# sjulier/Refactored_ORB_SLAM2

Measured on AMD Instinct MI355X. Metric: frames/s (extract+match) at KITTI 1241×376, 2000 feat; 1/2/4/8 GPU + CPU ref, higher is better.
Workload: dtype u8; 1 GPU; kitti_stereo_1241x376_2000feat_8lvl: 2x ORBextractor + ComputeStereoMatches + SearchByProjection(cur,last); parallelism=frame-shard x1, collective=none, driver=torch, queries=one pass: orbfe_track_queries_stereo_device

## Files before the change

refactored_orb_slam2_amd/csrc/match_kernels.hip:

```cpp
#include <string.h>
#include <atomic>
#include <mutex>

#include "match_internal.h"

#define WAVE 64

__device__ __forceinline__ int hamming256(const uint4 a0, const uint4 a1, const uint4 b0, const uint4 b1) {
  return __popc(a0.x ^ b0.x) + __popc(a0.y ^ b0.y) + __popc(a0.z ^ b0.z) + __popc(a0.w ^ b0.w) +
         __popc(a1.x ^ b1.x) + __popc(a1.y ^ b1.y) + __popc(a1.z ^ b1.z) + __popc(a1.w ^ b1.w);
}
__device__ __forceinline__ void load_desc(const uint8_t* p, uint4& d0, uint4& d1) {
  const uint4* q = reinterpret_cast<const uint4*>(p);
  d0 = q[0];
  d1 = q[1];
}
__device__ __forceinline__ void load_desc4(const uint8_t* p, uint4& d0, uint4& d1) {
  const uint32_t* q = reinterpret_cast<const uint32_t*>(p);
  d0 = make_uint4(q[0], q[1], q[2], q[3]);
  d1 = make_uint4(q[4], q[5], q[6], q[7]);
}

__device__ __forceinline__ unsigned wave_min_u32(unsigned v) {
#define ORBFE_MIN_STEP(ctrl, rmask) v = min(v, (unsigned)__builtin_amdgcn_update_dpp((int)0xffffffff, (int)v, ctrl, rmask, 0xf, false))
// ... 1089 lines not shown
      const int maxr = (int)ceilf(kp.y + r), minr = (int)floorf(kp.y - r);
      int b0 = max(minr, 0) >> 3, b1 = min(maxr >> 3, nb - 1);
      if (b1 - b0 >= STEREO_BUCKET_SPAN) b1 = b0 + STEREO_BUCKET_SPAN - 1;
      for (int b = b0; b <= b1; b++) {
        const int key = b * nl + oct;
        const int pos = atomicAdd(&cnt[key], 1);
        if (pass == 1) bi[start[key] + pos] = make_int4(iR, __float_as_int(kp.x), __float_as_int(kp.y), kp.octave);
      }
    }
    __syncthreads();
    if (pass == 0) {
      const int per = (nk + 255) / 256;
      const int k0 = min(tid * per, nk), k1 = min(k0 + per, nk);
      int sum = 0;
      for (int k = k0; k < k1; k++) sum += cnt[k];
      part[tid] = sum;
      __syncthreads();
      if (tid == 0) {
        int run = 0;
        for (int i = 0; i < 256; i++) { const int v = part[i]; part[i] = run; run += v; }
        start[nk] = run;
      }
      __syncthreads();
      int run = part[tid];
      for (int k = k0; k < k1; k++) { start[k] = run; run += cnt[k]; }
      __syncthreads();
      for (int b = tid; b <= nk; b += 256) bs[b] = start[b];
      for (int b = tid; b < nk; b += 256) cnt[b] = 0;
      __syncthreads();
    }
  }
}

__device__ __forceinline__ unsigned sad_u32(unsigned a, unsigned b, unsigned c) {
  unsigned r;
  asm("v_sad_u32 %0, %1, %2, %3" : "=v"(r) : "v"(a), "v"(b), "v"(c));
  return r;
}
#define ORBFE_ROW_ALL(op, v) do { \
    v = op(v, (unsigned)__builtin_amdgcn_update_dpp(0, (int)v, 0x128, 0xf, 0xf, false));  \
    v = op(v, (unsigned)__builtin_amdgcn_update_dpp(0, (int)v, 0x124, 0xf, 0xf, false));  \
    v = op(v, (unsigned)__builtin_amdgcn_update_dpp(0, (int)v, 0x122, 0xf, 0xf, false));  \
    v = op(v, (unsigned)__builtin_amdgcn_update_dpp(0, (int)v, 0x121, 0xf, 0xf, false));  \
  } while (0)
__device__ __forceinline__ unsigned op_min_u(unsigned a, unsigned b) { return min(a, b); }
__device__ __forceinline__ unsigned op_add_u(unsigned a, unsigned b) { return a + b; }
__device__ __forceinline__ unsigned op_or_u(unsigned a, unsigned b) { return a | b; }
__device__ __forceinline__ unsigned row_min_u32(unsigned v) { ORBFE_ROW_ALL(op_min_u, v); return v; }
__device__ __forceinline__ unsigned row_sum_u32(unsigned v) { ORBFE_ROW_ALL(op_add_u, v); return v; }
__device__ __forceinline__ unsigned row_or_u32(unsigned v) { ORBFE_ROW_ALL(op_or_u, v); return v; }

struct SmLevel {
  const uint8_t* baseL; const uint8_t* baseR;
  unsigned long long strideL, strideR;
  int pitchL, pitchR, wL, hL, wR, hR;
  float scale, inv_scale;
  int tiledL, tiledR;
};
#define SM_G 16
#define SM_KPB (256 / SM_G)
#ifndef SM_ROUNDS
#define SM_ROUNDS 2
#endif
#ifndef SM_SAD_T
#define SM_SAD_T 8
#endif
#define SAD_LP 32
#define SAD_RP 48
#define SAD_WIN (11 * SAD_LP + 11 * SAD_RP + 16)
#ifndef SM_XCD_PAIRS
#define SM_XCD_PAIRS 1
#endif
__global__ __launch_bounds__(256) void stereo_match_kernel(StereoParams P) {
  int pair = blockIdx.y, bx = blockIdx.x;
#if SM_XCD_PAIRS
  {
    const unsigned gx = gridDim.x;
    const unsigned lin = blockIdx.y * gx + blockIdx.x;
    const unsigned g8 = lin / (8u * gx);
    if (8u * g8 + 8u <= gridDim.y) {
      const unsigned within = lin - g8 * 8u * gx;
      pair = (int)(8u * g8 + (within & 7u));
      bx = (int)(within >> 3);
    }
  }
#endif
  const int lane = threadIdx.x & (WAVE - 1);
  const int sub = lane & (SM_G - 1);
  const int grp = threadIdx.x / SM_G;
  const int iL = bx * SM_KPB + grp;
  __shared__ SmLevel s_lv[ORBFE_MAX_LEVELS];
  __shared__ float s_r[ORBFE_MAX_LEVELS];
  __shared__ __attribute__((aligned(16))) uint8_t sad_win[SM_KPB][SAD_WIN];
  __shared__ uint16_t s_offL[128], s_offR[128];
  if (threadIdx.x >= 128) {
    const unsigned p = threadIdx.x - 128, yy = p / 11u, xx = p - yy * 11u;
    s_offL[p] = (uint16_t)(p < 121 ? yy * SAD_LP + xx : 0);
    s_offR[p] = (uint16_t)(p < 121 ? yy * SAD_RP + xx : 0);
  }
  if (threadIdx.x < ORBFE_MAX_LEVELS) {
    const int l = threadIdx.x;
    const bool in = l < P.n_levels;
    SmLevel v;
    v.baseL = P.pyrL.base[l] + (size_t)pair * P.pyrL.img_stride[l];
    v.baseR = P.pyrR.base[l] + (size_t)pair * P.pyrR.img_stride[l];
    v.strideL = 0; v.strideR = 0;
    v.pitchL = P.pyrL.pitch[l]; v.pitchR = P.pyrR.pitch[l];
    v.wL = in ? P.pyrL.w[l] : 0; v.hL = in ? P.pyrL.h[l] : 0;
    v.wR = in ? P.pyrR.w[l] : 0; v.hR = in ? P.pyrR.h[l] : 0;
    v.scale = P.scale[l]; v.inv_scale = P.inv_scale[l];
    v.tiledL = (int)((P.pyrL.tiled >> l) & 1u); v.tiledR = (int)((P.pyrR.tiled >> l) & 1u);
    s_lv[l] = v;
    s_r[l] = 2.0f * P.scale[l];
  }
  __syncthreads();
  const int cap = P.cap, nl = P.n_levels;
  float* out_ur = P.u_right + (size_t)pair * cap;
  float* out_depth = P.depth + (size_t)pair * cap;
  int32_t* out_sad = P.sad + (size_t)pair * cap;
  const orbfe_keypoint* kl = P.kpsL + (size_t)pair * cap;
  const uint8_t* dl = P.descL + (size_t)pair * cap * 32;
  const uint8_t* dr = P.descR + (size_t)pair * cap * 32;
  const int nL = P.nL[pair];
  const int iLc = min(iL, cap - 1);
  const float uL = kl[iLc].x, vL = kl[iLc].y;
  const int octL = kl[iLc].octave;
  uint4 a0, a1;
  load_desc(dl + (size_t)iLc * 32, a0, a1);
  if (sub == 0 && iL < cap) { out_ur[iL] = -1.0f; out_depth[iL] = -1.0f; out_sad[iL] = -1; }
  const int levelL = min(max(octL, 0), nl - 1);
  const int nRows = P.pyrL.h[0];
  const int row = (int)vL;
// ... 32 lines not shown
      if (__ballot(ok[r]) != 0ull) {
        const unsigned key = ((unsigned)hamming256(a0, a1, b0[r], b1[r]) << 16) | (unsigned)rec[r].x;
        if (ok[r] && key < best) {
          best = key;
          best_x = rx[r];
        }
      }
    }
  }
  {
    const unsigned k = ((best >> 16) < (unsigned)ORBFE_TH_HIGH) ? best : 0xFFFFFFFFu;
    best = row_min_u32(k);
    best_x = __int_as_float((int)row_or_u32((k == best && k != 0xFFFFFFFFu) ? (unsigned)__float_as_int(best_x) : 0u));
  }
  const float uR0 = best_x;
  const int thOrbDist = (ORBFE_TH_HIGH + ORBFE_TH_LOW) / 2;
  act = act && best != 0xFFFFFFFFu && (int)(best >> 16) < thOrbDist;
  if (__ballot(act) == 0ull) return;

  const SmLevel lv = s_lv[levelL];
  const float sfac = lv.inv_scale;
  const float scaleduL = roundf(uL * sfac);
  const float scaledvL = roundf(vL * sfac);
  const float scaleduR0 = roundf(uR0 * sfac);
  const int w = 5, L = 5;
  const float iniu = scaleduR0 + L - w;
  const float endu = scaleduR0 + L + w + 1;
  act = act && !(iniu < 0 || endu >= (float)lv.wR);
  const int yW = (int)(scaledvL - w), xW = (int)(scaleduL - w), xRc = (int)scaleduR0;
  const int xR0 = xRc - L - w;
  act = act && !(yW < 0 || yW + 2 * w >= lv.hL || xW < 0 || xW + 2 * w >= lv.wL || xR0 < 0 || xRc + L + w >= lv.wR ||
                 yW + 2 * w >= lv.hR);
  if (__ballot(act) == 0ull) return;
  uint8_t* winL = &sad_win[grp][0];
  uint8_t* winR = winL + 11 * SAD_LP;
  const int axL = xW & ~15, axR = xR0 & ~15;
  if (act && sub < 11) {
    typedef const __attribute__((address_space(1))) uint8_t* gptr_t;
    typedef unsigned int u32x4 __attribute__((ext_vector_type(4)));
    const int y = yW + sub;
    u32x4 vl[2], vr[3];
#pragma unroll
    for (int k = 0; k < 2; k++) {
      const int x = min(axL + 16 * k, lv.pitchL - 16);
      vl[k] = *reinterpret_cast<const __attribute__((address_space(1))) u32x4*>((gptr_t)(uintptr_t)lv.baseL + orbfe_level_offset(x, y, lv.pitchL, lv.tiledL != 0));
    }
#pragma unroll
    for (int k = 0; k < 3; k++) {
      const int x = min(axR + 16 * k, lv.pitchR - 16);
      vr[k] = *reinterpret_cast<const __attribute__((address_space(1))) u32x4*>((gptr_t)(uintptr_t)lv.baseR + orbfe_level_offset(x, y, lv.pitchR, lv.tiledR != 0));
    }
    u32x4* wl = reinterpret_cast<u32x4*>(winL + sub * SAD_LP);
    wl[0] = vl[0]; wl[1] = vl[1];
    u32x4* wr = reinterpret_cast<u32x4*>(winR + sub * SAD_RP);
    wr[0] = vr[0]; wr[1] = vr[1]; wr[2] = vr[2];
  }
  __builtin_amdgcn_fence(__ATOMIC_RELEASE, "wavefront");
  __builtin_amdgcn_wave_barrier();
  __builtin_amdgcn_fence(__ATOMIC_ACQUIRE, "wavefront");
  const uint8_t* WL = winL + (xW - axL);
  const uint8_t* WR = winR + (xR0 - axR);
  const int cLm = (int)WL[w * SAD_LP + w] - 255;
  int cRm[11];
#pragma unroll
  for (int k = 0; k < 11; k++) cRm[k] = (int)WR[w * SAD_RP + w + k] - 255;
  unsigned acc[11];
#pragma unroll
  for (int k = 0; k < 11; k++) acc[k] = 0;
#pragma unroll
  for (int t = 0; t < SM_SAD_T; t++) {
    const int p = sub + SM_G * t;
    if (t < 7 || p < 121) {
      const unsigned a = (unsigned)((int)WL[s_offL[p]] - cLm);
      const uint8_t* rrow = WR + s_offR[p];
#pragma unroll
      for (int k = 0; k < 11; k++) acc[k] = sad_u32(a, (unsigned)((int)rrow[k] - cRm[k]), acc[k]);
    }
  }
  unsigned pk[6];
#pragma unroll
  for (int j = 0; j < 5; j++) pk[j] = acc[2 * j] | (acc[2 * j + 1] << 16);
  pk[5] = acc[10];
#pragma unroll
  for (int j = 0; j < 6; j++) pk[j] = row_sum_u32(pk[j]);
  unsigned mine = pk[0];
  {
    const int t = sub >> 1;
    mine = t == 1 ? pk[1] : mine; mine = t == 2 ? pk[2] : mine; mine = t == 3 ? pk[3] : mine;
    mine = t == 4 ? pk[4] : mine; mine = t == 5 ? pk[5] : mine;
    mine = (sub & 1) ? (mine >> 16) : (mine & 0xffffu);
  }
  const unsigned kmin = row_min_u32(sub < 11 ? ((mine << 4) | (unsigned)sub) : 0xFFFFFFFFu);
  const int bk = (int)(kmin & 15u);
  const int sadBest = (int)(kmin >> 4);
  const int bestincR = bk - L;
  const int rowbase = lane & ~(SM_G - 1);
  const int i1 = __builtin_amdgcn_ds_bpermute((rowbase + ((bk + 15) & 15)) << 2, (int)mine);
  const int i3 = __builtin_amdgcn_ds_bpermute((rowbase + ((bk + 1) & 15)) << 2, (int)mine);
  const int i2 = sadBest;
  if (!act || sub != 0 || bestincR == -L || bestincR == L) return;
  const float dist1 = (float)i1, dist2 = (float)i2, dist3 = (float)i3;
  const float deltaR = (dist1 - dist3) / (2.0f * (dist1 + dist3 - 2.0f * dist2));
  if (deltaR < -1 || deltaR > 1) return;
  float bestuR = lv.scale * ((float)scaleduR0 + (float)bestincR + deltaR);
  float disparity = (uL - bestuR);
  if (disparity >= minD && disparity < maxD) {
    if (disparity <= 0) {
      disparity = (float)0.01;
      bestuR = (float)((double)uL - 0.01);
    }
    out_depth[iL] = P.mbf / disparity;
    out_ur[iL] = bestuR;
    out_sad[iL] = sadBest;
  }
}

__global__ __launch_bounds__(256) void stereo_median_kernel(StereoParams P) {
// ... 137 lines not shown
```

refactored_orb_slam2_amd/csrc/extract_kernels.hip:

```cpp
#include <stdlib.h>
#include <string.h>

#include "orbfe_internal.h"
#include "../../include/orb_pattern_data.h"

#define WAVE 64

__device__ __forceinline__ int wave_incl_scan(int v) {
  v += __builtin_amdgcn_update_dpp(0, v, 0x111, 0xf, 0xf, false);
  v += __builtin_amdgcn_update_dpp(0, v, 0x112, 0xf, 0xf, false);
  v += __builtin_amdgcn_update_dpp(0, v, 0x114, 0xf, 0xf, false);
  v += __builtin_amdgcn_update_dpp(0, v, 0x118, 0xf, 0xf, false);
  v += __builtin_amdgcn_update_dpp(0, v, 0x142, 0xa, 0xf, false);
  v += __builtin_amdgcn_update_dpp(0, v, 0x143, 0xc, 0xf, false);
  return v;
}

template <int T>
__device__ __forceinline__ int block_incl_scan_t(int v, int* tmp, int* total) {
  const int tid = threadIdx.x;
  const int lane = tid & (WAVE - 1), wid = tid >> 6;
  int s = wave_incl_scan(v);
  if (T == WAVE) {
    *total = __builtin_amdgcn_readlane(s, WAVE - 1);
// ... 2006 lines not shown
  }
  const double r = x * 0x1.45F306DC9C883p+23;
  const int n = ((int32_t)r + 0x800000) >> 24;
  x = x - (double)n * 0x1.921FB54442D18p0;
  const double s = ((n + 1) & 2) ? -1.0 : 1.0;
  const bool flip = (n & 2) != 0;
  const double xs = x * s, x2 = x * x;
  *sn = sc_poly(xs, x2, n, flip);
  *cs = sc_poly(xs, x2, n ^ 1, flip);
}

#ifndef ORI_PITCH
#define ORI_PITCH 48
#endif
#ifndef DSC_PITCH
#define DSC_PITCH 64
#endif
template <int PITCH>
__device__ __forceinline__ void patch_store16(uint8_t* base, int r, int c, const uint4& v) {
  if constexpr (PITCH % 16 == 0) {
    *reinterpret_cast<uint4*>(base + r * PITCH + 16 * c) = v;
  } else {
    uint32_t* q = reinterpret_cast<uint32_t*>(base + r * PITCH + 16 * c);
    q[0] = v.x; q[1] = v.y; q[2] = v.z; q[3] = v.w;
  }
}
#define ORI_BYTES ((31 * ORI_PITCH + 15) & ~15)
#ifndef OD_DMA_STAGE
#define OD_DMA_STAGE 1
#endif
#define OD_BUF (37 * DSC_PITCH)
#if OD_DMA_STAGE
#define PATCH_BYTES (2 * OD_BUF)
#define OD_DMA(gsrc, lds_dst) do { \
    unsigned keep_m0; \
    asm volatile("s_mov_b32 %0, m0\n\ts_mov_b32 m0, %2\n\ts_nop 0\n\tglobal_load_lds_dwordx4 %1, off\n\ts_mov_b32 m0, %0" \
                 : "=&s"(keep_m0) : "v"(gsrc), "s"(lds_dst) : "memory"); \
  } while (0)
#else
#define PATCH_BYTES ((ORI_BYTES + 37 * DSC_PITCH + 15) & ~15)
#endif

#ifndef OD_K
#define OD_K 8
#ifndef OD_DSC_NARROW
#define OD_DSC_NARROW 1
#endif
#endif
#ifndef OD_FAKE_TILED_RAW
#define OD_FAKE_TILED_RAW 0
#endif
#ifndef OD_FAKE_TABLES
#define OD_FAKE_TABLES 0
#endif
#if FC_TIMING
__device__ unsigned long long g_od_prof[4096 * 8];
extern "C" int orbfe_debug_od_profile(unsigned long long* out, int reset) {
  static unsigned long long h[4096 * 8];
  if (hipMemcpyFromSymbol(h, HIP_SYMBOL(g_od_prof), sizeof(h)) != hipSuccess) return 1;
  for (int i = 0; i < 8; i++) out[i] = 0;
  for (int sl = 0; sl < 4096; sl++)
    for (int i = 0; i < 8; i++) out[i] += h[sl * 8 + i];
  if (reset) { memset(h, 0, sizeof(h)); if (hipMemcpyToSymbol(HIP_SYMBOL(g_od_prof), h, sizeof(h)) != hipSuccess) return 1; }
  return 0;
}
#endif
__device__ __attribute__((aligned(16))) uint32_t g_ic_w[256 * 2];
#ifndef OD_WGS
#define OD_WGS 7
#endif
__global__ __launch_bounds__(256, OD_WGS) void orient_describe8_kernel(DescribeParams P) {
  __shared__ __attribute__((aligned(16))) uint8_t patch[4][PATCH_BYTES];
  const int lane = threadIdx.x & (WAVE - 1);
  const int wv_id = __builtin_amdgcn_readfirstlane((int)(threadIdx.x >> 6));
  int bx = blockIdx.x, img = blockIdx.y;
  if (P.xcd_images) {
    const unsigned gx = gridDim.x;
    const unsigned lin = blockIdx.y * gx + blockIdx.x;
    const unsigned grp = lin / (8u * gx);
    if (8u * grp + 8u <= gridDim.y) {
      const unsigned within = lin - grp * 8u * gx;
      img = (int)(8u * grp + (within & 7u));
      bx = (int)(within >> 3);
    }
  }
#if FC_TIMING
  uint32_t tacc0 = 0, tacc1 = 0, tacc2 = 0, tacc3 = 0, tacc4 = 0, tacc5 = 0, tprev = (uint32_t)__builtin_readcyclecounter();
#endif
  const int s0 = (bx * 4 + wv_id) * OD_K;
  const int32_t* ln = P.lvl_n + (size_t)img * ORBFE_MAX_LEVELS;
  if (s0 >= P.kp_per_image) return;
  const int ln_lane = lane < P.n_levels ? ln[lane] : 0;
  const int slot_c = min(s0 + (lane & (OD_K - 1)), P.kp_per_image - 1);
  const uint32_t e_lane = P.lvl_kp[(size_t)img * P.kp_per_image + slot_c];
  float4 pk[4];
#pragma unroll
#if OD_FAKE_TABLES
  for (int r = 0; r < 4; r++) pk[r] = make_float4((float)(lane & 7) - 3.f, (float)(r * 2 + (lane >> 4)) - 5.f, (float)(lane & 15) - 8.f, (float)(r) - 2.f);
#else
  for (int r = 0; r < 4; r++) pk[r] = *reinterpret_cast<const float4*>(&g_pattern_f[(r * 64 + lane) * 4]);
#endif
  uint32_t wu[4], wv[4];
#pragma unroll
  for (int j = 0; j < 4; j++) {
    const int it = lane + WAVE * j;
#if OD_FAKE_TABLES
    wu[j] = 0x01020304u * (uint32_t)(it & 7); wv[j] = 0x01010101u * (uint32_t)(it >> 3);
#else
    const uint2 w2 = reinterpret_cast<const uint2*>(g_ic_w)[it];
    wu[j] = w2.x; wv[j] = w2.y;
#endif
  }
#if !OD_DMA_STAGE
  uint8_t* ori = &patch[wv_id][0];
  uint8_t* dsc = ori + ORI_BYTES;
#endif

  int i_out = -1, i_level = 0, i_cx = 0, i_cy = 0, i_score = 0;
  {
    const int slot = s0 + lane;
    int level = 0, off_level = 0;
    for (int l = 1; l < P.n_levels; l++) {
      const bool ge = slot >= P.kp_off[l];
      level += ge ? 1 : 0;
      off_level = ge ? P.kp_off[l] : off_level;
    }
    const int idx = slot - off_level;
    int out = idx, ln_level = 0;
    for (int l = 0; l < P.n_levels; l++) {
      const int lnl = __builtin_amdgcn_readlane(ln_lane, l);
      out += l < level ? lnl : 0;
      ln_level = l == level ? lnl : ln_level;
    }
    if (lane < OD_K && slot < P.kp_per_image && idx < ln_level && out < P.cap) {
      const uint32_t e = e_lane;
      i_out = out; i_level = level;
      i_cx = (int)(e & 0xfff) + ORBFE_EDGE; i_cy = (int)((e >> 12) & 0xfff) + ORBFE_EDGE; i_score = (int)(e >> 24);
    }
    if (s0 == 0 && lane == 0) {
      int tot = 0;
      for (int l = 0; l < P.n_levels; l++) tot += __builtin_amdgcn_readlane(ln_lane, l);
      P.out_n[img] = tot;
    }
  }
  const unsigned valid_mask = (unsigned)(__ballot(i_out >= 0) & ((1ull << OD_K) - 1ull));
  if (valid_mask == 0) return;
  FC_T(0);

#if OD_DSC_NARROW && !OD_DMA_STAGE
  int r3[3], c3[3];
#pragma unroll
  for (int j = 0; j < 3; j++) { const int i = lane + WAVE * j; r3[j] = i / 3; c3[j] = i - 3 * r3[j]; }
#endif
#if !OD_DMA_STAGE
  auto issue_ori = [&](int k, uint4 vo[2]) {
    const int level = __builtin_amdgcn_readlane(i_level, k), cx = __builtin_amdgcn_readlane(i_cx, k), cy = __builtin_amdgcn_readlane(i_cy, k);
    const int pitch = P.pyr.pitch[level];
    const uint8_t* plane = P.pyr.base[level] + (size_t)img * P.pyr.img_stride[level];
    const int ax_o = (cx - 15) & ~15;
// ... 3 lines not shown
      const int r = i / 3, c = i - r * 3;
#if OD_FAKE_TILED_RAW
      (void)pitch; (void)plane;
      vo[j] = i < 31 * 3 ? *reinterpret_cast<const uint4*>(P.blur.base[level] + (size_t)img * P.blur.img_stride[level] + blur_tiled_offset(ax_o + 16 * c, cy - 15 + r, P.blur.pitch[level])) : make_uint4(0, 0, 0, 0);
#else
      vo[j] = i < 31 * 3 ? *reinterpret_cast<const uint4*>(plane + orbfe_level_offset(ax_o + 16 * c, cy - 15 + r, pitch, (P.pyr.tiled >> level) & 1u)) : make_uint4(0, 0, 0, 0);
#endif
    }
  };
  auto issue_dsc = [&](int k, uint4 vd[3]) {
    const int level = __builtin_amdgcn_readlane(i_level, k), cx = __builtin_amdgcn_readlane(i_cx, k), cy = __builtin_amdgcn_readlane(i_cy, k);
    const int bpitch = P.blur.pitch[level];
    const uint8_t* bplane = P.blur.base[level] + (size_t)img * P.blur.img_stride[level];
    const int ax_d = (cx - 18) & ~15;
#if OD_DSC_NARROW
    const bool wide = ((cx - 18) & 15) > 11;
    const int n_pieces = wide ? 37 * 4 : 37 * 3;
#pragma unroll
    for (int j = 0; j < 3; j++) {
      const int i = lane + WAVE * j;
      const int r = wide ? (i >> 2) : r3[j], c = wide ? (i & 3) : c3[j];
      vd[j] = i < n_pieces ? *reinterpret_cast<const uint4*>(bplane + blur_tiled_offset(max(ax_d + 16 * c, 0), max(cy - 18 + r, 0), bpitch)) : make_uint4(0, 0, 0, 0);
    }
#else
#pragma unroll
    for (int j = 0; j < 3; j++) {
      const int i = lane + WAVE * j;
      const int r = i >> 2, c = i & 3;
      vd[j] = i < 37 * 4 ? *reinterpret_cast<const uint4*>(bplane + blur_tiled_offset(max(ax_d + 16 * c, 0), max(cy - 18 + r, 0), bpitch)) : make_uint4(0, 0, 0, 0);
    }
#endif
  };
#endif
  auto next_valid = [&](int k) { const unsigned m = valid_mask >> (k + 1); return m ? k + 1 + (__ffs((int)m) - 1) : OD_K; };
  const int k_first = __ffs((int)valid_mask) - 1;

#if OD_DMA_STAGE
  const uint32_t lds_buf = (uint32_t)(uintptr_t)&patch[wv_id][0];
  auto dma_ori = [&](int k, uint32_t lds) {
    const int level = __builtin_amdgcn_readlane(i_level, k), cx = __builtin_amdgcn_readlane(i_cx, k), cy = __builtin_amdgcn_readlane(i_cy, k);
    const int pitch = P.pyr.pitch[level];
    const uint8_t* plane = P.pyr.base[level] + (size_t)img * P.pyr.img_stride[level];
    const bool tiled = (P.pyr.tiled >> level) & 1u;
    const int ax_o = (cx - 15) & ~15;
#pragma unroll
    for (int j = 0; j < 2; j++) {
      const int i = lane + WAVE * j;
      const int r = (i * 43) >> 7, c = i - 3 * r;
      if (i < 31 * 3) OD_DMA(plane + orbfe_level_offset(ax_o + 16 * c, cy - 15 + r, pitch, tiled), lds + 1024u * j);
    }
  };
  int m10v = 0, m01v = 0;
  {
    dma_ori(k_first, lds_buf);
    __builtin_amdgcn_s_waitcnt(0x0F70);
    uint32_t par = 0;
    for (int k = k_first; k < OD_K; k = next_valid(k), par ^= 1u) {
      const int kn = next_valid(k);
      if (kn < OD_K) {
        dma_ori(kn, lds_buf + (par ^ 1u) * OD_BUF);
        asm volatile("s_waitcnt vmcnt(2)" ::: "memory");
      } else {
        asm volatile("s_waitcnt vmcnt(0)" ::: "memory");
      }
      FC_T(1);
      const uint8_t* ob = &patch[wv_id][0] + par * OD_BUF;
      const int cx = __builtin_amdgcn_readlane(i_cx, k);
      const int m = (cx - 15) & 15;
      int A = 0, B = 0;
      const uint32_t sh = (uint32_t)(m & 3);
#pragma unroll
      for (int j = 0; j < 4; j++) {
        const int it = lane + WAVE * j;
        const int r = it >> 3, c = it & 7;
        const uint32_t* q = reinterpret_cast<const uint32_t*>(ob + (r < 31 ? r : 30) * ORI_PITCH + ((m + 4 * c) & ~3));
        const int px = (int)(__builtin_amdgcn_alignbyte(q[1], q[0], sh) ^ 0x80808080u);
        A = __builtin_amdgcn_sdot4(px, (int)wu[j], A, false);
        B = __builtin_amdgcn_sdot4(px, (int)wv[j], B, false);
      }
      const int At = __builtin_amdgcn_readlane(wave_incl_scan(A), 63), Bt = __builtin_amdgcn_readlane(wave_incl_scan(B), 63);
      if (lane == k) { m10v = At; m01v = Bt; }
      FC_T(2);
    }
  }
  auto dsc_wide = [&](int k) { return ((__builtin_amdgcn_readlane(i_cx, k) - 18) & 15) > 11; };
  auto dma_dsc = [&](int k, uint32_t lds) {
    const int level = __builtin_amdgcn_readlane(i_level, k), cx = __builtin_amdgcn_readlane(i_cx, k), cy = __builtin_amdgcn_readlane(i_cy, k);
    const int bpitch = P.blur.pitch[level];
    const uint8_t* bplane = P.blur.base[level] + (size_t)img * P.blur.img_stride[level];
    const int ax_d = (cx - 18) & ~15;
    const bool wide = ((cx - 18) & 15) > 11;
    const int n_pieces = wide ? 37 * 4 : 37 * 3;
#pragma unroll
    for (int j = 0; j < 3; j++) {
      const int i = lane + WAVE * j;
      const int q3 = (i * 43) >> 7;
      const int r = wide ? (i >> 2) : q3, c = wide ? (i & 3) : i - 3 * q3;
      if (j < 2 || wide)
        if (i < n_pieces) OD_DMA(bplane + blur_tiled_offset(max(ax_d + 16 * c, 0), max(cy - 18 + r, 0), bpitch), lds + 1024u * j);
    }
  };
  dma_dsc(k_first, lds_buf);
  const float angle_v = fast_atan2_deg((float)m01v, (float)m10v);
  const float factorPI = (float)(3.1415926535897932384626433832795 / 180.f);
  float a_v, b_v;
  glibc_sincosf(angle_v * factorPI, &b_v, &a_v);
  FC_T(3);
  {
    uint32_t par = 0;
    for (int k = k_first; k < OD_K; k = next_valid(k), par ^= 1u) {
      const int level = __builtin_amdgcn_readlane(i_level, k), cx = __builtin_amdgcn_readlane(i_cx, k), cy = __builtin_amdgcn_readlane(i_cy, k);
      const int out = __builtin_amdgcn_readlane(i_out, k), score = __builtin_amdgcn_readlane(i_score, k);
      const float a = __int_as_float(__builtin_amdgcn_readlane(__float_as_int(a_v), k)), b = __int_as_float(__builtin_amdgcn_readlane(__float_as_int(b_v), k)),
                  angle = __int_as_float(__builtin_amdgcn_readlane(__float_as_int(angle_v), k));
      const int ax_d = (cx - 18) & ~15;
      const bool wide = ((cx - 18) & 15) > 11;
      const int kn = next_valid(k);
      if (kn < OD_K) {
        dma_dsc(kn, lds_buf + (par ^ 1u) * OD_BUF);
        if (dsc_wide(kn)) asm volatile("s_waitcnt vmcnt(3)" ::: "memory");
        else asm volatile("s_waitcnt vmcnt(2)" ::: "memory");
      } else {
        asm volatile("s_waitcnt vmcnt(0)" ::: "memory");
      }
      FC_T(4);
      const uint8_t* dsc = &patch[wv_id][0] + par * OD_BUF;
      const float MAGIC = 12582912.0f;
      const uint32_t MB = 0x4B400000u;
      const uint32_t pitch = wide ? 64u : 48u;
      const uint32_t bc0 = 18u * pitch + (uint32_t)(cx - ax_d) - (MB * pitch + MB);
      uint8_t* dout = P.out_desc + ((size_t)img * P.cap + out) * 32;
      int t0[4], t1[4];
      if (wide) {
#pragma unroll
        for (int r = 0; r < 4; r++) {
          const float x0 = pk[r].x, y0 = pk[r].y, x1 = pk[r].z, y1 = pk[r].w;
          const uint32_t ry0 = __float_as_uint((x0 * b + y0 * a) + MAGIC), rx0 = __float_as_uint((x0 * a - y0 * b) + MAGIC);
          const uint32_t ry1 = __float_as_uint((x1 * b + y1 * a) + MAGIC), rx1 = __float_as_uint((x1 * a - y1 * b) + MAGIC);
          t0[r] = dsc[bc0 + ry0 * 64u + rx0];
          t1[r] = dsc[bc0 + ry1 * 64u + rx1];
        }
      } else {
#pragma unroll
        for (int r = 0; r < 4; r++) {
          const float x0 = pk[r].x, y0 = pk[r].y, x1 = pk[r].z, y1 = pk[r].w;
          const uint32_t ry0 = __float_as_uint((x0 * b + y0 * a) + MAGIC), rx0 = __float_as_uint((x0 * a - y0 * b) + MAGIC);
          const uint32_t ry1 = __float_as_uint((x1 * b + y1 * a) + MAGIC), rx1 = __float_as_uint((x1 * a - y1 * b) + MAGIC);
          t0[r] = dsc[bc0 + ry0 * 48u + rx0];
          t1[r] = dsc[bc0 + ry1 * 48u + rx1];
        }
      }
      {
        const unsigned long long b0 = __ballot(t0[0] < t1[0]), b1 = __ballot(t0[1] < t1[1]), b2 = __ballot(t0[2] < t1[2]), b3 = __ballot(t0[3] < t1[3]);
        const unsigned long long mine = lane == 0 ? b0 : lane == 1 ? b1 : lane == 2 ? b2 : b3;
        if (lane < 4) reinterpret_cast<unsigned long long*>(dout)[lane] = mine;
      }
      {
        float fx = (float)cx, fy = (float)cy;
        if (level != 0) {
          fx *= P.scale[level];
          fy *= P.scale[level];
        }
        uint32_t wvv;
        switch (lane) {
          case 0: wvv = __float_as_uint(fx); break;
          case 1: wvv = __float_as_uint(fy); break;
          case 2: wvv = __float_as_uint(P.kp_size[level]); break;
          case 3: wvv = __float_as_uint(angle); break;
          case 4: wvv = __float_as_uint((float)score); break;
          case 5: wvv = (uint32_t)level; break;
          default: wvv = 0xFFFFFFFFu; break;
        }
        if (lane < 7) reinterpret_cast<uint32_t*>(P.out_kps + (size_t)img * P.cap + out)[lane] = wvv;
      }
      FC_T(5);
    }
  }
#else
  int m10v = 0, m01v = 0;
  {
    uint4 vn[2];
    issue_ori(k_first, vn);
    for (int k = k_first; k < OD_K; k = next_valid(k)) {
      const int cx = __builtin_amdgcn_readlane(i_cx, k);
      const int m = (cx - 15) & 15;
#pragma unroll
      for (int j = 0; j < 2; j++) {
        const int i = lane + WAVE * j;
        const int r = i / 3, c = i - r * 3;
        if (i < 31 * 3) patch_store16<ORI_PITCH>(ori, r, c, vn[j]);
      }
      FC_T(1);
      const int kn = next_valid(k);
      if (kn < OD_K) issue_ori(kn, vn);
      __builtin_amdgcn_fence(__ATOMIC_RELEASE, "wavefront");
      __builtin_amdgcn_wave_barrier();
      __builtin_amdgcn_fence(__ATOMIC_ACQUIRE, "wavefront");
      int A = 0, B = 0;
      const uint32_t sh = (uint32_t)(m & 3);
#pragma unroll
      for (int j = 0; j < 4; j++) {
        const int it = lane + WAVE * j;
        const int r = it >> 3, c = it & 7;
        const uint32_t* q = reinterpret_cast<const uint32_t*>(ori + (r < 31 ? r : 30) * ORI_PITCH + ((m + 4 * c) & ~3));
        const int px = (int)(__builtin_amdgcn_alignbyte(q[1], q[0], sh) ^ 0x80808080u);
        A = __builtin_amdgcn_sdot4(px, (int)wu[j], A, false);
        B = __builtin_amdgcn_sdot4(px, (int)wv[j], B, false);
      }
      const int At = __builtin_amdgcn_readlane(wave_incl_scan(A), 63), Bt = __builtin_amdgcn_readlane(wave_incl_scan(B), 63);
      if (lane == k) { m10v = At; m01v = Bt; }
// ... 231 lines not shown
```

Before: 112,800 frames/s.

## Compute stereo SAD from registers with packed u16 SAD, dropping LDS window

Stereo SAD refinement no longer stages the 11x11 left and 11x21 right windows in shared memory. Each lane keeps one image row in vector registers, extracts byte pairs with perm/alignbyte, and accumulates two pixels at a time with v_sad_u16, with center bias broadcast through ds_bpermute. The tiled address computation is inlined, and the extra right and left loads are skipped when the aligned window fits in fewer 16-byte chunks. This removes LDS traffic, the offset tables and the wave barrier, at the cost of more register pressure and fragile byte-select arithmetic.

```diff
diff --git a/refactored_orb_slam2_amd/csrc/match_kernels.hip b/refactored_orb_slam2_amd/csrc/match_kernels.hip
--- a/refactored_orb_slam2_amd/csrc/match_kernels.hip
+++ b/refactored_orb_slam2_amd/csrc/match_kernels.hip
@@ -1145,9 +1145,9 @@
   }
 }
 
-__device__ __forceinline__ unsigned sad_u32(unsigned a, unsigned b, unsigned c) {
+__device__ __forceinline__ unsigned sad_u16(unsigned a, unsigned b, unsigned c) {
   unsigned r;
-  asm("v_sad_u32 %0, %1, %2, %3" : "=v"(r) : "v"(a), "v"(b), "v"(c));
+  asm("v_sad_u16 %0, %1, %2, %3" : "=v"(r) : "v"(a), "v"(b), "v"(c));
   return r;
 }
 #define ORBFE_ROW_ALL(op, v) do { \
@@ -1175,12 +1175,6 @@
 #ifndef SM_ROUNDS
 #define SM_ROUNDS 2
 #endif
-#ifndef SM_SAD_T
-#define SM_SAD_T 8
-#endif
-#define SAD_LP 32
-#define SAD_RP 48
-#define SAD_WIN (11 * SAD_LP + 11 * SAD_RP + 16)
 #ifndef SM_XCD_PAIRS
 #define SM_XCD_PAIRS 1
 #endif
@@ -1204,13 +1198,6 @@
   const int iL = bx * SM_KPB + grp;
   __shared__ SmLevel s_lv[ORBFE_MAX_LEVELS];
   __shared__ float s_r[ORBFE_MAX_LEVELS];
-  __shared__ __attribute__((aligned(16))) uint8_t sad_win[SM_KPB][SAD_WIN];
-  __shared__ uint16_t s_offL[128], s_offR[128];
-  if (threadIdx.x >= 128) {
-    const unsigned p = threadIdx.x - 128, yy = p / 11u, xx = p - yy * 11u;
-    s_offL[p] = (uint16_t)(p < 121 ? yy * SAD_LP + xx : 0);
-    s_offR[p] = (uint16_t)(p < 121 ? yy * SAD_RP + xx : 0);
-  }
   if (threadIdx.x < ORBFE_MAX_LEVELS) {
     const int l = threadIdx.x;
     const bool in = l < P.n_levels;
@@ -1309,57 +1296,72 @@
   act = act && !(yW < 0 || yW + 2 * w >= lv.hL || xW < 0 || xW + 2 * w >= lv.wL || xR0 < 0 || xRc + L + w >= lv.wR ||
                  yW + 2 * w >= lv.hR);
   if (__ballot(act) == 0ull) return;
-  uint8_t* winL = &sad_win[grp][0];
-  uint8_t* winR = winL + 11 * SAD_LP;
+  typedef unsigned int u32x4 __attribute__((ext_vector_type(4)));
   const int axL = xW & ~15, axR = xR0 & ~15;
+  const unsigned oL = (unsigned)(xW - axL), oR = (unsigned)(xR0 - axR);
+  u32x4 vl0, vl1, vr0, vr1, vr2;
+  asm("" : "=v"(vl0), "=v"(vl1), "=v"(vr0), "=v"(vr1), "=v"(vr2));
   if (act && sub < 11) {
     typedef const __attribute__((address_space(1))) uint8_t* gptr_t;
-    typedef unsigned int u32x4 __attribute__((ext_vector_type(4)));
-    const int y = yW + sub;
-    u32x4 vl[2], vr[3];
-#pragma unroll
-    for (int k = 0; k < 2; k++) {
-      const int x = min(axL + 16 * k, lv.pitchL - 16);
-      vl[k] = *reinterpret_cast<const __attribute__((address_space(1))) u32x4*>((gptr_t)(uintptr_t)lv.baseL + orbfe_level_offset(x, y, lv.pitchL, lv.tiledL != 0));
-    }
-#pragma unroll
-    for (int k = 0; k < 3; k++) {
-      const int x = min(axR + 16 * k, lv.pitchR - 16);
-      vr[k] = *reinterpret_cast<const __attribute__((address_space(1))) u32x4*>((gptr_t)(uintptr_t)lv.baseR + orbfe_level_offset(x, y, lv.pitchR, lv.tiledR != 0));
-    }
-    u32x4* wl = reinterpret_cast<u32x4*>(winL + sub * SAD_LP);
-    wl[0] = vl[0]; wl[1] = vl[1];
-    u32x4* wr = reinterpret_cast<u32x4*>(winR + sub * SAD_RP);
-    wr[0] = vr[0]; wr[1] = vr[1]; wr[2] = vr[2];
-  }
-  __builtin_amdgcn_fence(__ATOMIC_RELEASE, "wavefront");
-  __builtin_amdgcn_wave_barrier();
-  __builtin_amdgcn_fence(__ATOMIC_ACQUIRE, "wavefront");
-  const uint8_t* WL = winL + (xW - axL);
-  const uint8_t* WR = winR + (xR0 - axR);
-  const int cLm = (int)WL[w * SAD_LP + w] - 255;
-  int cRm[11];
-#pragma unroll
-  for (int k = 0; k < 11; k++) cRm[k] = (int)WR[w * SAD_RP + w + k] - 255;
+    typedef const __attribute__((address_space(1))) u32x4* gvec_t;
+    const unsigned y = (unsigned)(yW + sub), ty = (y & 7u) << 4;
+    const bool tL = lv.tiledL != 0, tR = lv.tiledR != 0;
+    const unsigned pL = (unsigned)lv.pitchL, pR = (unsigned)lv.pitchR;
+    const unsigned offL = tL ? ((((y >> 3) * (pL >> 4) + ((unsigned)axL >> 4)) << 7) | ty) : y * pL + (unsigned)axL;
+    const unsigned offR = tR ? ((((y >> 3) * (pR >> 4) + ((unsigned)axR >> 4)) << 7) | ty) : y * pR + (unsigned)axR;
+    const unsigned stepL = tL ? 128u : 16u, stepR = tR ? 128u : 16u;
+    const gptr_t bL = (gptr_t)(uintptr_t)lv.baseL, bR = (gptr_t)(uintptr_t)lv.baseR;
+    vl0 = *reinterpret_cast<gvec_t>(bL + offL);
+    if (oL > 16 - 11) vl1 = *reinterpret_cast<gvec_t>(bL + (offL + stepL));
+    vr0 = *reinterpret_cast<gvec_t>(bR + offR);
+    vr1 = *reinterpret_cast<gvec_t>(bR + (offR + stepR));
+    if (oR > 32 - 21) vr2 = *reinterpret_cast<gvec_t>(bR + (offR + 2u * stepR));
+  }
+  const bool l1 = (oL & 4u) != 0, l2 = (oL & 8u) != 0, r1 = (oR & 4u) != 0, r2 = (oR & 8u) != 0;
+  const unsigned tl0 = l2 ? vl0.z : vl0.x, tl1 = l2 ? vl0.w : vl0.y, tl2 = l2 ? vl1.x : vl0.z, tl3 = l2 ? vl1.y : vl0.w,
+                 tl4 = l2 ? vl1.z : vl1.x;
+  const unsigned ql[4] = {l1 ? tl1 : tl0, l1 ? tl2 : tl1, l1 ? tl3 : tl2, l1 ? tl4 : tl3};
+  const unsigned tr0 = r2 ? vr0.z : vr0.x, tr1 = r2 ? vr0.w : vr0.y, tr2 = r2 ? vr1.x : vr0.z, tr3 = r2 ? vr1.y : vr0.w,
+                 tr4 = r2 ? vr1.z : vr1.x, tr5 = r2 ? vr1.w : vr1.y, tr6 = r2 ? vr2.x : vr1.z;
+  const unsigned qr[6] = {r1 ? tr1 : tr0, r1 ? tr2 : tr1, r1 ? tr3 : tr2, r1 ? tr4 : tr3, r1 ? tr5 : tr4, r1 ? tr6 : tr5};
+  const unsigned shL = (oL & 3u) * 0x00010001u, shR = (oR & 3u) * 0x00010001u;
+  const unsigned selL0 = 0x0c010c00u + shL, selL2 = 0x0c030c02u + shL;
+  const unsigned selR[4] = {0x0c010c00u + shR, 0x0c020c01u + shR, 0x0c030c02u + shR, 0x0c040c03u + shR};
+  const int src5 = ((lane & ~(SM_G - 1)) + 5) << 2;
+  const unsigned biasL = (unsigned)__builtin_amdgcn_ds_bpermute(src5, (int)__builtin_amdgcn_perm(ql[2], ql[1], 0x0c010c01u + shL)) ^ 0x00ff00ffu;
+  unsigned nc[3];
+#pragma unroll
+  for (int i = 0; i < 3; i++)
+    nc[i] = (unsigned)__builtin_amdgcn_ds_bpermute(src5, (int)~__builtin_amdgcn_alignbyte(qr[i + 2], qr[i + 1], oR & 3u));
+  unsigned D[11];
+#pragma unroll
+  for (int k = 0; k < 11; k++) {
+    const unsigned bsel = (unsigned)((5 + k) & 3);
+    D[k] = __builtin_amdgcn_perm(0u, nc[(5 + k - 4) >> 2], 0x0c000c00u | (bsel << 16) | bsel);
+  }
+  unsigned A[6];
+#pragma unroll
+  for (int j = 0; j < 5; j++) A[j] = __builtin_amdgcn_perm(ql[(j >> 1) + 1], ql[j >> 1], (j & 1) ? selL2 : selL0) + biasL;
+  A[5] = __builtin_amdgcn_perm(ql[3], ql[2], 0x0c0c0c02u + (oL & 3u)) + (biasL & 0xffffu);
   unsigned acc[11];
 #pragma unroll
   for (int k = 0; k < 11; k++) acc[k] = 0;
 #pragma unroll
-  for (int t = 0; t < SM_SAD_T; t++) {
-    const int p = sub + SM_G * t;
-    if (t < 7 || p < 121) {
-      const unsigned a = (unsigned)((int)WL[s_offL[p]] - cLm);
-      const uint8_t* rrow = WR + s_offR[p];
-#pragma unroll
-      for (int k = 0; k < 11; k++) acc[k] = sad_u32(a, (unsigned)((int)rrow[k] - cRm[k]), acc[k]);
-    }
+  for (int m = 0; m < 21; m++) {
+    const unsigned R = __builtin_amdgcn_perm(qr[min((m >> 2) + 1, 5)], qr[m >> 2], selR[m & 3]);
+#pragma unroll
+    for (int j = 0; j < 5; j++) {
+      const int k = m - 2 * j;
+      if (k >= 0 && k < 11) acc[k] = sad_u16(A[j], R + D[k], acc[k]);
+    }
+    if (m >= 10) acc[m - 10] = sad_u16(A[5], (R + D[m - 10]) & 0xffffu, acc[m - 10]);
   }
   unsigned pk[6];
 #pragma unroll
   for (int j = 0; j < 5; j++) pk[j] = acc[2 * j] | (acc[2 * j + 1] << 16);
   pk[5] = acc[10];
 #pragma unroll
-  for (int j = 0; j < 6; j++) pk[j] = row_sum_u32(pk[j]);
+  for (int j = 0; j < 6; j++) pk[j] = row_sum_u32(sub < 11 ? pk[j] : 0u);
   unsigned mine = pk[0];
   {
     const int t = sub >> 1;
```

Result: no change. 113,300 frames/s (median of 6 runs) (+0.4%).

## Precompute per-lane DMA addressing and restructure orientation reduction in orient_describe kernel

Applied to the files above, without the earlier changes.

Per-keypoint plane bases, pitches and tiling terms are now computed once per lane up front, and each DMA step pulls them with readlane. This replaces the per-iteration scalar loads and the generic offset function. The DMA uses the SGPR base plus VGPR offset form and masks the tail with exec instead of per-lane branches. The full-wave moment scan per keypoint becomes a partial DPP reduction, with one cross-row finish after the loop. Keypoint record stores move out of the loop into one per-lane write, and the wide/narrow descriptor sampling paths merge through a umul24 pitch. This adds inline-asm m0/exec handling with hand-picked nop counts, and changes how the reduction result is assigned to lanes, which could be subtly wrong.

```diff
diff --git a/refactored_orb_slam2_amd/csrc/extract_kernels.hip b/refactored_orb_slam2_amd/csrc/extract_kernels.hip
--- a/refactored_orb_slam2_amd/csrc/extract_kernels.hip
+++ b/refactored_orb_slam2_amd/csrc/extract_kernels.hip
@@ -2062,10 +2062,12 @@
 #define OD_BUF (37 * DSC_PITCH)
 #if OD_DMA_STAGE
 #define PATCH_BYTES (2 * OD_BUF)
-#define OD_DMA(gsrc, lds_dst) do { \
-    unsigned keep_m0; \
-    asm volatile("s_mov_b32 %0, m0\n\ts_mov_b32 m0, %2\n\ts_nop 0\n\tglobal_load_lds_dwordx4 %1, off\n\ts_mov_b32 m0, %0" \
-                 : "=&s"(keep_m0) : "v"(gsrc), "s"(lds_dst) : "memory"); \
+#define OD_DMA_S(voff, sbase, lds_dst) \
+    asm volatile("s_mov_b32 m0, %2\n\ts_nop 3\n\tglobal_load_lds_dwordx4 %0, %1" : : "v"(voff), "s"(sbase), "s"(lds_dst) : "memory")
+#define OD_DMA_SM(voff, sbase, lds_dst, mask) do { \
+    unsigned long long keep_exec; \
+    asm volatile("s_mov_b32 m0, %3\n\ts_nop 2\n\ts_and_saveexec_b64 %0, %4\n\tglobal_load_lds_dwordx4 %1, %2\n\ts_mov_b64 exec, %0" \
+                 : "=&s"(keep_exec) : "v"(voff), "s"(sbase), "s"(lds_dst), "s"(mask) : "memory", "scc"); \
   } while (0)
 #else
 #define PATCH_BYTES ((ORI_BYTES + 37 * DSC_PITCH + 15) & ~15)
@@ -2082,6 +2084,12 @@
 #endif
 #ifndef OD_FAKE_TABLES
 #define OD_FAKE_TABLES 0
+#endif
+#ifndef OD_SCAN6
+#define OD_SCAN6 0
+#endif
+#ifndef OD_BOUND
+#define OD_BOUND 0
 #endif
 #if FC_TIMING
 __device__ unsigned long long g_od_prof[4096 * 8];
@@ -2147,6 +2155,12 @@
 #endif
 
   int i_out = -1, i_level = 0, i_cx = 0, i_cy = 0, i_score = 0;
+#if OD_DMA_STAGE
+  unsigned long long pl_rbase, pl_bbase;
+  int pl_rpitch, pl_bpitch;
+  uint32_t pl_rtiled;
+  float pl_scale, pl_size;
+#endif
   {
     const int slot = s0 + lane;
     int level = 0, off_level = 0;
@@ -2155,6 +2169,16 @@
       level += ge ? 1 : 0;
       off_level = ge ? P.kp_off[l] : off_level;
     }
+#if OD_DMA_STAGE
+    const int lq = OD_BOUND ? 0 : level;
+    pl_rbase = reinterpret_cast<unsigned long long>(P.pyr.base[lq]) + (unsigned long long)img * P.pyr.img_stride[lq];
+    pl_bbase = reinterpret_cast<unsigned long long>(P.blur.base[lq]) + (unsigned long long)img * P.blur.img_stride[lq];
+    pl_rpitch = P.pyr.pitch[lq];
+    pl_bpitch = P.blur.pitch[lq];
+    pl_rtiled = (P.pyr.tiled >> lq) & 1u;
+    pl_scale = P.scale[level];
+    pl_size = P.kp_size[level];
+#endif
     const int idx = slot - off_level;
     int out = idx, ln_level = 0;
     for (int l = 0; l < P.n_levels; l++) {
@@ -2224,32 +2248,50 @@
 #endif
   };
 #endif
+  const int k_first = __ffs((int)valid_mask) - 1;
+#if !OD_DMA_STAGE
   auto next_valid = [&](int k) { const unsigned m = valid_mask >> (k + 1); return m ? k + 1 + (__ffs((int)m) - 1) : OD_K; };
-  const int k_first = __ffs((int)valid_mask) - 1;
+#endif
 
 #if OD_DMA_STAGE
+  const uint32_t r_mA = pl_rtiled ? (uint32_t)(pl_rpitch >> 4) << 7 : (uint32_t)pl_rpitch << 3;
+  const uint32_t r_mB = pl_rtiled ? 16u : (uint32_t)pl_rpitch;
+  const uint32_t r_cs = pl_rtiled ? 128u : 16u;
+  const unsigned long long r_base = pl_rbase + (unsigned long long)((uint32_t)((i_cx - 15) >> 4) * r_cs);
+  const int r_blo = (int)(uint32_t)r_base, r_bhi = (int)(uint32_t)(r_base >> 32);
+  const int r_y0 = i_cy - 15;
+  const int r_m = (i_cx - 15) & 15;
+  const int b_lo = (int)(uint32_t)pl_bbase, b_hi = (int)(uint32_t)(pl_bbase >> 32);
+  const uint32_t b_mA = (uint32_t)(pl_bpitch >> 4) << 7;
+  const int b_x16 = (i_cx - 18) >> 4, b_y0 = i_cy - 18;
+  const int b_wide = ((i_cx - 18) & 15) > 11 ? 1 : 0;
+  const int rN0 = (lane * 43) >> 7, cN0 = lane - 3 * rN0;
+  const int rN1 = ((lane + WAVE) * 43) >> 7, cN1 = lane + WAVE - 3 * rN1;
+  const int rW = lane >> 2, cW = lane & 3;
+#define OD_RL(v, k) __builtin_amdgcn_readlane((v), (k))
+#define OD_RL64(lo, hi, k) (((unsigned long long)(uint32_t)OD_RL(hi, k) << 32) | (unsigned long long)(uint32_t)OD_RL(lo, k))
   const uint32_t lds_buf = (uint32_t)(uintptr_t)&patch[wv_id][0];
   auto dma_ori = [&](int k, uint32_t lds) {
-    const int level = __builtin_amdgcn_readlane(i_level, k), cx = __builtin_amdgcn_readlane(i_cx, k), cy = __builtin_amdgcn_readlane(i_cy, k);
-    const int pitch = P.pyr.pitch[level];
-    const uint8_t* plane = P.pyr.base[level] + (size_t)img * P.pyr.img_stride[level];
-    const bool tiled = (P.pyr.tiled >> level) & 1u;
-    const int ax_o = (cx - 15) & ~15;
-#pragma unroll
-    for (int j = 0; j < 2; j++) {
-      const int i = lane + WAVE * j;
-      const int r = (i * 43) >> 7, c = i - 3 * r;
-      if (i < 31 * 3) OD_DMA(plane + orbfe_level_offset(ax_o + 16 * c, cy - 15 + r, pitch, tiled), lds + 1024u * j);
-    }
+    const unsigned long long base = OD_RL64(r_blo, r_bhi, k);
+    const uint32_t mA = (uint32_t)OD_RL((int)r_mA, k), mB = (uint32_t)OD_RL((int)r_mB, k), cs = (uint32_t)OD_RL((int)r_cs, k);
+    const int y0 = OD_RL(r_y0, k);
+    const uint32_t ya = (uint32_t)(y0 + rN0), yb = (uint32_t)(y0 + rN1);
+    const uint32_t oa = __umul24(ya >> 3, mA) + __umul24(ya & 7u, mB) + __umul24((uint32_t)cN0, cs);
+    const uint32_t ob = __umul24(yb >> 3, mA) + __umul24(yb & 7u, mB) + __umul24((uint32_t)cN1, cs);
+    OD_DMA_S(oa, base, lds);
+    OD_DMA_SM(ob, base, lds + 1024u, (1ull << (31 * 3 - WAVE)) - 1ull);
   };
-  int m10v = 0, m01v = 0;
+  int accA = 0, accB = 0;
   {
     dma_ori(k_first, lds_buf);
     __builtin_amdgcn_s_waitcnt(0x0F70);
+    unsigned rem = valid_mask & (valid_mask - 1u);
     uint32_t par = 0;
-    for (int k = k_first; k < OD_K; k = next_valid(k), par ^= 1u) {
-      const int kn = next_valid(k);
-      if (kn < OD_K) {
+    for (int k = k_first;; par ^= 1u) {
+      const int kn = __builtin_ctz(rem | (1u << OD_K));
+      const bool more = kn < OD_K;
+      rem &= rem - 1u;
+      if (more) {
         dma_ori(kn, lds_buf + (par ^ 1u) * OD_BUF);
         asm volatile("s_waitcnt vmcnt(2)" ::: "memory");
       } else {
@@ -2257,8 +2299,7 @@
       }
       FC_T(1);
       const uint8_t* ob = &patch[wv_id][0] + par * OD_BUF;
-      const int cx = __builtin_amdgcn_readlane(i_cx, k);
-      const int m = (cx - 15) & 15;
+      const int m = OD_RL(r_m, k);
       int A = 0, B = 0;
       const uint32_t sh = (uint32_t)(m & 3);
 #pragma unroll
@@ -2270,104 +2311,121 @@
         A = __builtin_amdgcn_sdot4(px, (int)wu[j], A, false);
         B = __builtin_amdgcn_sdot4(px, (int)wv[j], B, false);
       }
-      const int At = __builtin_amdgcn_readlane(wave_incl_scan(A), 63), Bt = __builtin_amdgcn_readlane(wave_incl_scan(B), 63);
-      if (lane == k) { m10v = At; m01v = Bt; }
+#if OD_SCAN6
+      A = __builtin_amdgcn_readlane(wave_incl_scan(A), 63);
+      B = __builtin_amdgcn_readlane(wave_incl_scan(B), 63);
+#elif !OD_BOUND
+      A += __builtin_amdgcn_update_dpp(0, A, 0xB1, 0xf, 0xf, false);
+      B += __builtin_amdgcn_update_dpp(0, B, 0xB1, 0xf, 0xf, false);
+      A += __builtin_amdgcn_update_dpp(0, A, 0x4E, 0xf, 0xf, false);
+      B += __builtin_amdgcn_update_dpp(0, B, 0x4E, 0xf, 0xf, false);
+      A += __builtin_amdgcn_update_dpp(0, A, 0x141, 0xf, 0xf, false);
+      B += __builtin_amdgcn_update_dpp(0, B, 0x141, 0xf, 0xf, false);
+#endif
+      const bool mine = (lane & 7) == k;
+      accA = mine ? A : accA;
+      accB = mine ? B : accB;
       FC_T(2);
-    }
-  }
-  auto dsc_wide = [&](int k) { return ((__builtin_amdgcn_readlane(i_cx, k) - 18) & 15) > 11; };
-  auto dma_dsc = [&](int k, uint32_t lds) {
-    const int level = __builtin_amdgcn_readlane(i_level, k), cx = __builtin_amdgcn_readlane(i_cx, k), cy = __builtin_amdgcn_readlane(i_cy, k);
-    const int bpitch = P.blur.pitch[level];
-    const uint8_t* bplane = P.blur.base[level] + (size_t)img * P.blur.img_stride[level];
-    const int ax_d = (cx - 18) & ~15;
-    const bool wide = ((cx - 18) & 15) > 11;
-    const int n_pieces = wide ? 37 * 4 : 37 * 3;
-#pragma unroll
-    for (int j = 0; j < 3; j++) {
-      const int i = lane + WAVE * j;
-      const int q3 = (i * 43) >> 7;
-      const int r = wide ? (i >> 2) : q3, c = wide ? (i & 3) : i - 3 * q3;
-      if (j < 2 || wide)
-        if (i < n_pieces) OD_DMA(bplane + blur_tiled_offset(max(ax_d + 16 * c, 0), max(cy - 18 + r, 0), bpitch), lds + 1024u * j);
+      if (!more) break;
+      k = kn;
+    }
+  }
+  auto dma_dsc = [&](int k, uint32_t lds, bool wide) {
+    const unsigned long long base = OD_RL64(b_lo, b_hi, k);
+    const uint32_t mA = (uint32_t)OD_RL((int)b_mA, k);
+    const int x16 = OD_RL(b_x16, k), y0 = OD_RL(b_y0, k);
+    const uint32_t xc = (uint32_t)max(x16 + (wide ? cW : cN0), 0), xd = (uint32_t)max(x16 + (wide ? cW : cN1), 0);
+    const uint32_t ya = (uint32_t)max(y0 + (wide ? rW : rN0), 0), yb = (uint32_t)max(y0 + (wide ? rW + 16 : rN1), 0);
+    const uint32_t oa = __umul24(ya >> 3, mA) + ((ya & 7u) << 4) + (xc << 7);
+    const uint32_t ob = __umul24(yb >> 3, mA) + ((yb & 7u) << 4) + (xd << 7);
+    OD_DMA_S(oa, base, lds);
+    OD_DMA_SM(ob, base, lds + 1024u, wide ? ~0ull : (1ull << (37 * 3 - WAVE)) - 1ull);
+    if (wide) {
+      const uint32_t ye = (uint32_t)max(y0 + rW + 32, 0);
+      const uint32_t oe = __umul24(ye >> 3, mA) + ((ye & 7u) << 4) + (xc << 7);
+      OD_DMA_SM(oe, base, lds + 2048u, (1ull << (37 * 4 - 2 * WAVE)) - 1ull);
     }
   };
-  dma_dsc(k_first, lds_buf);
+  bool wide_k = OD_RL(b_wide, k_first) != 0;
+  dma_dsc(k_first, lds_buf, wide_k);
+  accA += __builtin_amdgcn_update_dpp(0, accA, 0x128, 0xf, 0xf, false);
+  accB += __builtin_amdgcn_update_dpp(0, accB, 0x128, 0xf, 0xf, false);
+  accA += __builtin_amdgcn_ds_bpermute((lane ^ 16) << 2, accA);
+  accB += __builtin_amdgcn_ds_bpermute((lane ^ 16) << 2, accB);
+  accA += __builtin_amdgcn_ds_bpermute((lane ^ 32) << 2, accA);
+  accB += __builtin_amdgcn_ds_bpermute((lane ^ 32) << 2, accB);
+  const int m10v = accA, m01v = accB;
   const float angle_v = fast_atan2_deg((float)m01v, (float)m10v);
   const float factorPI = (float)(3.1415926535897932384626433832795 / 180.f);
   float a_v, b_v;
   glibc_sincosf(angle_v * factorPI, &b_v, &a_v);
+  if (i_out >= 0) {
+    float fx = (float)i_cx, fy = (float)i_cy;
+    if (i_level != 0) {
+      fx *= pl_scale;
+      fy *= pl_scale;
+    }
+    uint32_t* o = reinterpret_cast<uint32_t*>(P.out_kps + (size_t)img * P.cap + i_out);
+    o[0] = __float_as_uint(fx);
+    o[1] = __float_as_uint(fy);
+    o[2] = __float_as_uint(pl_size);
+    o[3] = __float_as_uint(angle_v);
+    o[4] = __float_as_uint((float)i_score);
+    o[5] = (uint32_t)i_level;
+    o[6] = 0xFFFFFFFFu;
+  }
+  const uint32_t MB = 0x4B400000u;
+  const uint32_t d_pitch = b_wide ? 64u : 48u;
+  const uint32_t d_bc = 18u * d_pitch + 18u + (uint32_t)((i_cx - 18) & 15) - ((1u << 22) * d_pitch + MB);
+  const unsigned long long d_out = ((unsigned long long)img * (unsigned)P.cap + (unsigned)max(i_out, 0)) * 32ull;
+  const int d_olo = (int)(uint32_t)d_out, d_ohi = (int)(uint32_t)(d_out >> 32);
   FC_T(3);
   {
+    const float MAGIC = 12582912.0f;
+    const uint32_t sel0 = lane == 0 ? ~0u : 0u, sel1 = lane == 1 ? ~0u : 0u, sel2 = lane == 2 ? ~0u : 0u, sel3 = lane == 3 ? ~0u : 0u;
+    unsigned rem = valid_mask & (valid_mask - 1u);
     uint32_t par = 0;
-    for (int k = k_first; k < OD_K; k = next_valid(k), par ^= 1u) {
-      const int level = __builtin_amdgcn_readlane(i_level, k), cx = __builtin_amdgcn_readlane(i_cx, k), cy = __builtin_amdgcn_readlane(i_cy, k);
-      const int out = __builtin_amdgcn_readlane(i_out, k), score = __builtin_amdgcn_readlane(i_score, k);
-      const float a = __int_as_float(__builtin_amdgcn_readlane(__float_as_int(a_v), k)), b = __int_as_float(__builtin_amdgcn_readlane(__float_as_int(b_v), k)),
-                  angle = __int_as_float(__builtin_amdgcn_readlane(__float_as_int(angle_v), k));
-      const int ax_d = (cx - 18) & ~15;
-      const bool wide = ((cx - 18) & 15) > 11;
-      const int kn = next_valid(k);
-      if (kn < OD_K) {
-        dma_dsc(kn, lds_buf + (par ^ 1u) * OD_BUF);
-        if (dsc_wide(kn)) asm volatile("s_waitcnt vmcnt(3)" ::: "memory");
+    for (int k = k_first;; par ^= 1u) {
+      const int kn = __builtin_ctz(rem | (1u << OD_K));
+      const bool more = kn < OD_K;
+      rem &= rem - 1u;
+      const float a = __int_as_float(OD_RL(__float_as_int(a_v), k)), b = __int_as_float(OD_RL(__float_as_int(b_v), k));
+      const uint32_t pitch = wide_k ? 64u : 48u;
+      if (more) {
+        wide_k = OD_RL(b_wide, kn) != 0;
+        dma_dsc(kn, lds_buf + (par ^ 1u) * OD_BUF, wide_k);
+        if (wide_k) asm volatile("s_waitcnt vmcnt(3)" ::: "memory");
         else asm volatile("s_waitcnt vmcnt(2)" ::: "memory");
       } else {
         asm volatile("s_waitcnt vmcnt(0)" ::: "memory");
       }
       FC_T(4);
       const uint8_t* dsc = &patch[wv_id][0] + par * OD_BUF;
-      const float MAGIC = 12582912.0f;
-      const uint32_t MB = 0x4B400000u;
-      const uint32_t pitch = wide ? 64u : 48u;
-      const uint32_t bc0 = 18u * pitch + (uint32_t)(cx - ax_d) - (MB * pitch + MB);
-      uint8_t* dout = P.out_desc + ((size_t)img * P.cap + out) * 32;
+      const uint32_t bc0 = (uint32_t)OD_RL((int)d_bc, k);
+      uint2* dout = reinterpret_cast<uint2*>(P.out_desc + OD_RL64(d_olo, d_ohi, k));
       int t0[4], t1[4];
-      if (wide) {
-#pragma unroll
-        for (int r = 0; r < 4; r++) {
-          const float x0 = pk[r].x, y0 = pk[r].y, x1 = pk[r].z, y1 = pk[r].w;
-          const uint32_t ry0 = __float_as_uint((x0 * b + y0 * a) + MAGIC), rx0 = __float_as_uint((x0 * a - y0 * b) + MAGIC);
-          const uint32_t ry1 = __float_as_uint((x1 * b + y1 * a) + MAGIC), rx1 = __float_as_uint((x1 * a - y1 * b) + MAGIC);
-          t0[r] = dsc[bc0 + ry0 * 64u + rx0];
-          t1[r] = dsc[bc0 + ry1 * 64u + rx1];
-        }
-      } else {
-#pragma unroll
-        for (int r = 0; r < 4; r++) {
-          const float x0 = pk[r].x, y0 = pk[r].y, x1 = pk[r].z, y1 = pk[r].w;
-          const uint32_t ry0 = __float_as_uint((x0 * b + y0 * a) + MAGIC), rx0 = __float_as_uint((x0 * a - y0 * b) + MAGIC);
-          const uint32_t ry1 = __float_as_uint((x1 * b + y1 * a) + MAGIC), rx1 = __float_as_uint((x1 * a - y1 * b) + MAGIC);
-          t0[r] = dsc[bc0 + ry0 * 48u + rx0];
-          t1[r] = dsc[bc0 + ry1 * 48u + rx1];
-        }
+#pragma unroll
+      for (int r = 0; r < 4; r++) {
+        const float x0 = pk[r].x, y0 = pk[r].y, x1 = pk[r].z, y1 = pk[r].w;
+        const uint32_t ry0 = __float_as_uint((x0 * b + y0 * a) + MAGIC), rx0 = __float_as_uint((x0 * a - y0 * b) + MAGIC);
+        const uint32_t ry1 = __float_as_uint((x1 * b + y1 * a) + MAGIC), rx1 = __float_as_uint((x1 * a - y1 * b) + MAGIC);
+        t0[r] = dsc[bc0 + __umul24(ry0, pitch) + rx0];
+        t1[r] = dsc[bc0 + __umul24(ry1, pitch) + rx1];
       }
       {
         const unsigned long long b0 = __ballot(t0[0] < t1[0]), b1 = __ballot(t0[1] < t1[1]), b2 = __ballot(t0[2] < t1[2]), b3 = __ballot(t0[3] < t1[3]);
-        const unsigned long long mine = lane == 0 ? b0 : lane == 1 ? b1 : lane == 2 ? b2 : b3;
-        if (lane < 4) reinterpret_cast<unsigned long long*>(dout)[lane] = mine;
-      }
-      {
-        float fx = (float)cx, fy = (float)cy;
-        if (level != 0) {
-          fx *= P.scale[level];
-          fy *= P.scale[level];
-        }
-        uint32_t wvv;
-        switch (lane) {
-          case 0: wvv = __float_as_uint(fx); break;
-          case 1: wvv = __float_as_uint(fy); break;
-          case 2: wvv = __float_as_uint(P.kp_size[level]); break;
-          case 3: wvv = __float_as_uint(angle); break;
-          case 4: wvv = __float_as_uint((float)score); break;
-          case 5: wvv = (uint32_t)level; break;
-          default: wvv = 0xFFFFFFFFu; break;
-        }
-        if (lane < 7) reinterpret_cast<uint32_t*>(P.out_kps + (size_t)img * P.cap + out)[lane] = wvv;
+        uint2 mine;
+        mine.x = ((uint32_t)b0 & sel0) | ((uint32_t)b1 & sel1) | ((uint32_t)b2 & sel2) | ((uint32_t)b3 & sel3);
+        mine.y = ((uint32_t)(b0 >> 32) & sel0) | ((uint32_t)(b1 >> 32) & sel1) | ((uint32_t)(b2 >> 32) & sel2) | ((uint32_t)(b3 >> 32) & sel3);
+        if (lane < 4) dout[lane] = mine;
       }
       FC_T(5);
-    }
-  }
+      if (!more) break;
+      k = kn;
+    }
+  }
+#undef OD_RL
+#undef OD_RL64
 #else
   int m10v = 0, m01v = 0;
   {
```

Result: faster. 112,500 frames/s before, 113,800 frames/s after (median of 6 runs) (+1.2%).
